# WeiZhang1988/YDORBSLAM

Hardware: AMD Instinct MI355X
Metric: ORB extract+match Mkeypoints/sec (higher is better)
Workload: dtype u8

## Files before the change

### ydorbslam_amd/csrc/match_kernels.hip.h

```cpp
#pragma once
#include <hip/hip_runtime.h>
#include <stdint.h>

#include <type_traits>

#include "grid_build.hip.h"

#pragma clang fp contract(off)

namespace ydorb {

constexpr int kHistLen = 30, kThHigh = 100, kThLow = 50;

template <class T> using gptr = __attribute__((address_space(1))) T*;
template <class T> __device__ __forceinline__ gptr<T> G(T* p) { return (gptr<T>)p; }

struct QueryDev {
  float u, v, r;
  int minLevel, maxLevel;
  float ur, rs, angle;
  int level, flags;
};

__global__ __launch_bounds__(256) void k_grid_build(const FrameDev* __restrict__ frames, int cap) {
  __shared__ int hist[kGridCells];
  __shared__ int wsum[4];
  extern __shared__ int16_t cellOf[];
  const FrameDev F = frames[blockIdx.x];
  grid_build<true>(F, cap, hist, wsum, cellOf);
}

__device__ __forceinline__ int hamming256(const uint8_t* a, const uint8_t* b) {
  const uint4 a0 = *reinterpret_cast<const uint4*>(a), a1 = *reinterpret_cast<const uint4*>(a + 16);
  const uint4 b0 = *reinterpret_cast<const uint4*>(b), b1 = *reinterpret_cast<const uint4*>(b + 16);
  return __popc(a0.x ^ b0.x) + __popc(a0.y ^ b0.y) + __popc(a0.z ^ b0.z) + __popc(a0.w ^ b0.w) + __popc(a1.x ^ b1.x) +
         __popc(a1.y ^ b1.y) + __popc(a1.z ^ b1.z) + __popc(a1.w ^ b1.w);
}

struct CallDev {
  int frame;
  const KeyPointDev* tkps;
  const float* qAngle;
  const QueryDev* queries;
  const uint8_t* qdesc;
  const int* nqPtr;
  int nq;
  int2* qInfo;
  uint8_t* taken;
  int* assigned;
  int* matchQ;
  int* count;
  int mode;
  float ratio;
  int orbDist, checkOri;
  float invSigma2[8];
  const KeyPointDev* qkps;
  uint2* qPre;
  int takenClear;
};
__device__ __forceinline__ int call_nq(const CallDev& C) { return C.nqPtr ? *C.nqPtr : C.nq; }

__device__ __forceinline__ unsigned wave_min_u32(unsigned v) {
#define YD_DPP_MIN(ctrl, rmask) v = min(v, (unsigned)__builtin_amdgcn_update_dpp((int)v, (int)v, ctrl, rmask, 0xF, false))
  YD_DPP_MIN(0xB1, 0xF);
  YD_DPP_MIN(0x4E, 0xF);
  YD_DPP_MIN(0x141, 0xF);
  YD_DPP_MIN(0x140, 0xF);
  YD_DPP_MIN(0x142, 0xA);
  YD_DPP_MIN(0x143, 0xC);
#undef YD_DPP_MIN
  return (unsigned)__builtin_amdgcn_readlane((int)v, 63);
}

constexpr int kSlot = 64;
#ifndef GATHER_QPW
#define GATHER_QPW 1
#endif
constexpr int kGatherQpw = GATHER_QPW;
__global__ __launch_bounds__(256) void k_gather_projection(const CallDev* __restrict__ calls, const FrameDev* __restrict__ frames,
                                                           int maxQ, uint32_t* __restrict__ pool, unsigned* __restrict__ poolHeads,
                                                           unsigned poolPerCall, int* __restrict__ status) {
  __shared__ int pref[4][64];
  __shared__ int sStart[4][64];
  const int lane = threadIdx.x & 63, wv = threadIdx.x >> 6;
  const int q0 = (blockIdx.x * 4 + wv) * kGatherQpw;
  const CallDev C = calls[blockIdx.y];
  const int nqAll = min(maxQ, call_nq(C));
  if (q0 >= nqAll) return;
  const FrameDev F = frames[C.frame];
  QueryDev Qs[kGatherQpw];
#pragma unroll
  for (int i = 0; i < kGatherQpw; i++) Qs[i] = C.queries[min(q0 + i, nqAll - 1)];
  struct Window { bool ok; int nx, start, cnt; };
  auto window = [&](const QueryDev& Q) -> Window {
    Window W{false, 0, 0, 0};
    if (!(Q.flags & 1)) return W;
    const int minCellX = max(0, (int)floorf(__fmul_rn(__fsub_rn(__fsub_rn(Q.u, F.minX), Q.r), F.gridWInv)));
    const int maxCellX = min(kGridCols - 1, (int)ceilf(__fmul_rn(__fadd_rn(__fsub_rn(Q.u, F.minX), Q.r), F.gridWInv)));
    const int minCellY = max(0, (int)floorf(__fmul_rn(__fsub_rn(__fsub_rn(Q.v, F.minY), Q.r), F.gridHInv)));
    const int maxCellY = min(kGridRows - 1, (int)ceilf(__fmul_rn(__fadd_rn(__fsub_rn(Q.v, F.minY), Q.r), F.gridHInv)));
    if (!(minCellX < kGridCols && maxCellX >= 0 && minCellY < kGridRows && maxCellY >= 0 && minCellX <= maxCellX && minCellY <= maxCellY)) return W;
    W.ok = true;
    W.nx = maxCellX - minCellX + 1;
    if (lane < W.nx) {
      const int c0 = (minCellX + lane) * kGridRows;
      W.start = F.cellStart[c0 + minCellY];
      W.cnt = F.cellStart[c0 + maxCellY + 1] - W.start;
    }
    return W;
  };
  Window Wn = window(Qs[0]);
#pragma unroll
  for (int qi = 0; qi < kGatherQpw; qi++) {
  const int q = q0 + qi;
  if (q >= nqAll) break;
  const QueryDev Q = Qs[qi];
  const Window Wc = Wn;
  if (qi + 1 < kGatherQpw && q + 1 < nqAll) Wn = window(Qs[qi + 1]);
  int2 info = make_int2(0, 0);
  if (Wc.ok) {
    {
      const int nx = Wc.nx;
      const int start = Wc.start, cnt = Wc.cnt;
      int incl = cnt;
#pragma unroll
      for (int d = 1; d < 64; d <<= 1) { const int y = __shfl_up(incl, d, 64); if (lane >= d) incl += y; }
      const int total = __shfl(incl, 63, 64);
      if (total > 0) {
        pref[wv][lane] = incl;
        sStart[wv][lane] = start;
        __builtin_amdgcn_wave_barrier();
        auto staticTest = [&](int t, int& pos, int& idx) -> bool {
          int lo = 0, hi = nx - 1;
          while (lo < hi) { const int mid = (lo + hi) >> 1; if (pref[wv][mid] > t) hi = mid; else lo = mid + 1; }
          pos = sStart[wv][lo] + (t - (lo ? pref[wv][lo - 1] : 0));
          const float4 kp = F.sortedKp[pos];
          const int octave = __float_as_int(kp.z);
          idx = __float_as_int(kp.w);
          bool pass = true;
          if (Q.minLevel > 0 || Q.maxLevel >= 0)
            if (octave < Q.minLevel || (Q.maxLevel >= 0 && octave < Q.maxLevel)) pass = false;
          if (!(fabsf(__fsub_rn(kp.x, Q.u)) > Q.r && fabsf(__fsub_rn(kp.y, Q.v)) < Q.r)) pass = false;
          if (pass && C.mode == 6) {
            const float rx = F.rightX ? F.rightX[idx] : -1.0f;
            const double ax = (double)__fsub_rn(kp.x, Q.u), ay = (double)__fsub_rn(kp.y, Q.v), ar = (double)__fsub_rn(rx, Q.ur);
            const float monoErr = (float)(ax * ax + ay * ay);
            const float stereoErr = (float)((double)monoErr + ar * ar);
            const bool lv = octave >= Q.level - 1 && octave <= Q.level;
            const float is2 = calls[blockIdx.y].invSigma2[octave & 7];
            pass = lv && ((rx >= 0 && (double)__fmul_rn(stereoErr, is2) <= 7.81) || (rx < 0 && (double)__fmul_rn(monoErr, is2) <= 5.99));
          } else if (pass && C.mode == 7) {
            pass = octave >= Q.level - 1 && octave <= Q.level;
          } else if (pass && C.mode != 2 && F.rightX) {
            const float rx = F.rightX[idx];
            if (!(rx <= 0 || fabsf(__fsub_rn(Q.ur, rx)) <= Q.rs)) pass = false;
          }
          return pass;
        };
        int need = total;
        if (total > kSlot) {
          need = 0;
          for (int t0 = 0; t0 < total; t0 += 64) {
            const int t = t0 + lane;
            int pos, idx;
            const bool pass = t < total && staticTest(t, pos, idx);
            need += __popcll(__ballot(pass));
          }
        }
        unsigned base;
        bool ok = true;
        if (need <= kSlot) {
          base = blockIdx.y * poolPerCall + (unsigned)q * kSlot;
        } else {
          unsigned off = 0;
          if (lane == 0) off = atomicAdd(poolHeads + blockIdx.y, (unsigned)need);
          off = __shfl(off, 0, 64);
          const unsigned ovfBase = (unsigned)maxQ * kSlot;
          ok = ovfBase + off + (unsigned)need <= poolPerCall;
          base = blockIdx.y * poolPerCall + ovfBase + off;
          if (!ok && lane == 0) atomicMax(status, 1);
        }
        if (ok && need > 0) {
          int written = 0;
          unsigned k1 = 0xFFFFFFFFu, k2 = 0xFFFFFFFFu, r1 = 0, r2 = 0;
          const bool pre = C.qPre != nullptr, readTaken = pre && C.taken && !C.takenClear;
          const uint4* qd = reinterpret_cast<const uint4*>(C.qdesc + (size_t)q * 32);
          const uint4 qa = qd[0], qb = qd[1];
          for (int t0 = 0; t0 < total; t0 += 64) {
            const int t = t0 + lane;
            int pos = 0, idx = 0, dist = 0;
            const bool pass = t < total && staticTest(t, pos, idx);
            if (pass) {
              const uint4* td = reinterpret_cast<const uint4*>(F.sortedDesc + (size_t)pos * 32);
              const uint4 ta = td[0], tb = td[1];
              dist = __popc(qa.x ^ ta.x) + __popc(qa.y ^ ta.y) + __popc(qa.z ^ ta.z) + __popc(qa.w ^ ta.w) + __popc(qb.x ^ tb.x) +
                     __popc(qb.y ^ tb.y) + __popc(qb.z ^ tb.z) + __popc(qb.w ^ tb.w);
            }
            const unsigned long long m = __ballot(pass);
            if (pass) {
              const int wpos = written + __popcll(m & ((1ull << lane) - 1ull));
              const uint32_t rec = ((uint32_t)dist << 16) | (uint32_t)idx;
              pool[base + wpos] = rec;
              if (pre && !(readTaken && C.taken[idx])) {
                const unsigned key = ((unsigned)dist << 23) | (unsigned)wpos;
                if (key < k1) { k2 = k1; r2 = r1; k1 = key; r1 = rec; } else if (key < k2) { k2 = key; r2 = rec; }
              }
            }
            written += __popcll(m);
          }
          if (pre) {
            const unsigned b1 = wave_min_u32(k1);
            const bool own = k1 == b1 && b1 != 0xFFFFFFFFu;
            const unsigned long long o1 = __ballot(own);
            const unsigned br = o1 ? (unsigned)__builtin_amdgcn_readlane((int)r1, (int)__builtin_ctzll(o1)) : 0xFFFFFFFFu;
            if (own) { k1 = k2; r1 = r2; }
            const unsigned b2 = wave_min_u32(k1);
            const unsigned long long o2 = __ballot(k1 == b2 && b2 != 0xFFFFFFFFu);
            const unsigned sr = o2 ? (unsigned)__builtin_amdgcn_readlane((int)r1, (int)__builtin_ctzll(o2)) : 0xFFFFFFFFu;
            if (lane == 0) C.qPre[q] = make_uint2(o1 ? br : 0xFFFFFFFFu, sr);
          }
          info = make_int2((int)base, written);
        }
      }
    }
  }
  if (lane == 0) C.qInfo[q] = info;
  __builtin_amdgcn_wave_barrier();
  }
}

struct BowCallDev {
  const uint8_t* descA; const uint8_t* descB;
  const int* qFeat; const int2* qRange; const int* featB; const uint8_t* validB;
  int nq;
  int2* qInfo;
  int tri;
  const KeyPointDev* kpsA; const KeyPointDev* kpsB;
  const uint8_t* goodA; const uint8_t* goodB;
  float F[9], ex, ey, sfB[8], sf2B[8];
};
__device__ __forceinline__ bool tri_pair_ok(const BowCallDev& B, const KeyPointDev& k1, bool good1, const KeyPointDev& k2, bool good2) {
  if (!(good1 || good2)) {
    const float dx = __fsub_rn(B.ex, k2.x), dy = __fsub_rn(B.ey, k2.y);
    const double far = (double)dx * (double)dx + (double)dy * (double)dy;
    if (!(far >= (double)__fmul_rn(100.0f, B.sfB[k2.octave]))) return false;
  }
  const float la = __fadd_rn(__fadd_rn(__fmul_rn(B.F[0], k1.x), __fmul_rn(B.F[3], k1.y)), B.F[6]);
  const float lb = __fadd_rn(__fadd_rn(__fmul_rn(B.F[1], k1.x), __fmul_rn(B.F[4], k1.y)), B.F[7]);
  const float lc = __fadd_rn(__fadd_rn(__fmul_rn(B.F[2], k1.x), __fmul_rn(B.F[5], k1.y)), B.F[8]);
  const float den = __fadd_rn(__fmul_rn(la, la), __fmul_rn(lb, lb));
  if (!(den > 0.0f)) return false;
  const float num = __fadd_rn(__fadd_rn(__fmul_rn(la, k2.x), __fmul_rn(lb, k2.y)), lc);
  return (double)__fdiv_rn(__fmul_rn(num, num), __fmul_rn(den, den)) < 3.841 * (double)B.sf2B[k2.octave];
}
__global__ __launch_bounds__(256) void k_gather_bow(BowCallDev B, uint32_t* __restrict__ pool, unsigned* __restrict__ poolHead,
                                                    unsigned poolCap, int* __restrict__ status) {
  const int lane = threadIdx.x & 63, wv = threadIdx.x >> 6;
  const int q = blockIdx.x * 4 + wv;
  if (q >= B.nq) return;
  const int2 rg = B.qRange[q];
  const int total = rg.y - rg.x;
  int2 info = make_int2(0, 0);
  if (total > 0) {
    unsigned base = 0;
    if (lane == 0) base = atomicAdd(poolHead, (unsigned)total);
    base = __shfl(base, 0, 64);
    if (base + (unsigned)total > poolCap) {
      if (lane == 0) atomicMax(status, 1);
    } else {
      const uint8_t* qd = B.descA + (size_t)B.qFeat[q] * 32;
      int written = 0;
      for (int t0 = 0; t0 < total; t0 += 64) {
        const int t = t0 + lane;
        bool pass = false;
        int idx = 0, dist = 0;
        if (t < total) {
          idx = B.featB[rg.x + t];
          pass = !B.validB || B.validB[idx];
          if (pass) dist = hamming256(qd, B.descB + (size_t)idx * 32);
          if (pass && B.tri) {
            const int i1 = B.qFeat[q];
            pass = dist <= kThLow && tri_pair_ok(B, B.kpsA[i1], B.goodA[i1] != 0, B.kpsB[idx], B.goodB[idx] != 0);
          }
        }
        const unsigned long long m = __ballot(pass);
        if (pass) pool[base + written + __popcll(m & ((1ull << lane) - 1ull))] = ((uint32_t)dist << 16) | (uint32_t)idx;
        written += __popcll(m);
      }
      info = make_int2((int)base, written);
    }
  }
  if (lane == 0) B.qInfo[q] = info;
}


__global__ __launch_bounds__(256) void k_distinctive(const uint8_t* __restrict__ desc, const int* __restrict__ offsets, int nPoints,
                                                     int* __restrict__ best) {
  const int p = blockIdx.x * 4 + (threadIdx.x >> 6), lane = threadIdx.x & 63;
  if (p >= nPoints) return;
  const int o0 = __builtin_amdgcn_readfirstlane(offsets[p]), m = __builtin_amdgcn_readfirstlane(offsets[p + 1]) - o0;
  if (m <= 0) { if (lane == 0) best[p] = -1; return; }
  const uint8_t* D = desc + (size_t)o0 * 32;
  const int kth = (int)(0.5 * m);
  unsigned win = 0xFFFFFFFFu;
  for (int i0 = 0; i0 < m; i0 += 64) {
    const int i = i0 + lane;
    if (i < m) {
      const uint4 a0 = *reinterpret_cast<const uint4*>(D + (size_t)i * 32), a1 = *reinterpret_cast<const uint4*>(D + (size_t)i * 32 + 16);
      int lo = 0, hi = 256;
      while (lo < hi) {
// ... 403 lines not shown
```

### ydorbslam_amd/csrc/orb_matcher.hip

```cpp
#include <hip/hip_runtime.h>

#include <algorithm>
#include <cstdlib>
#include <cmath>
#include <cstring>
#include <vector>

#include "../../include/ydorb/c_api.h"
#include "frustum_kernels.hip.h"
#include "host_buffers.h"
#include "match_kernels.hip.h"
#include "stereo_kernels.hip.h"
#include "ydorb_host.h"

using namespace ydorb;

namespace {

int launchGridBuild(int nFrames, int cap, hipStream_t s, const FrameDev* frames) {
  const size_t dyn = sizeof(int16_t) * (size_t)std::max(cap, 0);
  if (dyn > 48 * 1024)
    HIPCHK(hipFuncSetAttribute(reinterpret_cast<const void*>(k_grid_build), hipFuncAttributeMaxDynamicSharedMemorySize, (int)dyn));
  hipLaunchKernelGGL(k_grid_build, dim3(nFrames), dim3(256), dyn, s, frames, cap);
  HIPCHK(hipGetLastError());
// ... 35 lines not shown
struct ProjPtrs {
  int* status; FrameDev* frame; CallDev* call;
  KeyPointDev* kps; uint8_t* desc; float* rightX; int *cellStart, *cellIdx; float4* sortedKp; uint8_t* sortedDesc;
  QueryDev* queries; uint8_t *qdesc, *taken; int *assigned, *matchQ; int2* qInfo; uint2* qPre;
  uint8_t *table, *track;
};
size_t layProjection(size_t n, bool stereo, size_t nq, size_t tableBytes, size_t trackBytes, void* base, ProjPtrs& p) {
  Carve a(base);
  a.take(p.status, 16); a.take(p.frame, 1); a.take(p.call, 1);
  a.take(p.kps, n); a.take(p.desc, 32 * n); a.take(p.rightX, stereo ? n : 0); a.take(p.cellStart, kGridCells + 1); a.take(p.cellIdx, n);
  a.take(p.sortedKp, n); a.take(p.sortedDesc, 32 * n);
  a.take(p.queries, nq); a.take(p.qdesc, 32 * nq); a.take(p.taken, n + kTakenPad); a.take(p.assigned, n); a.take(p.matchQ, nq); a.take(p.qInfo, nq);
  a.take(p.qPre, nq); a.take(p.table, tableBytes); a.take(p.track, trackBytes);
  return a.L.bytes;
}

struct BowPtrs {
  int* status; CallDev* call;
  uint8_t *descA, *descB, *valid, *goodA, *goodB; KeyPointDev *kpsA, *kpsB; int *feat, *qFeat, *assigned, *matchQ; int2 *qRange, *qInfo; float* qAngle;
};
size_t layBow(size_t nA, size_t nB, size_t nFeatB, size_t nq, bool tri, void* base, BowPtrs& p) {
  Carve a(base);
  a.take(p.status, 16); a.take(p.call, 1);
  a.take(p.descA, 32 * nA); a.take(p.descB, 32 * nB); a.take(p.kpsB, nB); a.take(p.feat, nFeatB); a.take(p.valid, nB);
  a.take(p.qFeat, nq); a.take(p.qRange, nq); a.take(p.qAngle, nq); a.take(p.qInfo, nq); a.take(p.matchQ, nq); a.take(p.assigned, std::max(nq, nB));
  a.take(p.kpsA, tri ? nA : 0); a.take(p.goodA, tri ? nA : 0); a.take(p.goodB, tri ? nB : 0);
  return a.L.bytes;
}

struct RowsPtrs { uint8_t *a, *b; int *offsets, *idx, *out; TopkOut* top; };
size_t layRows(size_t nA, size_t nB, size_t nOffsets, size_t nIdx, size_t nOut, size_t nTop, void* base, RowsPtrs& r) {
  Carve a(base);
  a.take(r.a, 32 * nA); a.take(r.b, 32 * nB); a.take(r.offsets, nOffsets); a.take(r.idx, nIdx); a.take(r.out, nOut); a.take(r.top, nTop);
  return a.L.bytes;
}

struct StereoPtrs { int *counters, *kept, *status, *nL, *nR; KeyPointDev *kpsL, *kpsR; uint8_t *descL, *descR; float *rightX, *depth; };
size_t layStereo(size_t nPairs, size_t nl, size_t nr, void* base, StereoPtrs& p) {
  Carve a(base);
  a.take(p.counters, 4 * nPairs); a.take(p.kept, nPairs); a.take(p.status, nPairs);
  a.take(p.kpsL, nl); a.take(p.descL, 32 * nl); a.take(p.kpsR, nr); a.take(p.descR, 32 * nr); a.take(p.nL, nl ? nPairs : 0); a.take(p.nR, nl ? nPairs : 0);
  a.take(p.rightX, nl); a.take(p.depth, nl);
  return a.L.bytes;
}

}

struct ydorb_matcher {
  int device = 0;
  hipStream_t stream = nullptr;
  Mem call;
  Mem pool;
  size_t poolRecords = 1u << 20;
  Mem stereo;
  PinnedMem hUp, hDown;
  struct Batch {
    Mem arena;
    Mem status;
    std::vector<FrameDev> hFrames;
    std::vector<CallDev> hCalls;
    float hSf[8] = {0};
    bool hIdentAffine = false;
    BatchPtrs at{};
    int ovfPerKeypoint = 16;
  } batch;
  bool profiling = false;
  hipEvent_t ev[MS_COUNT + 1]{};
  double stageMs[MS_COUNT]{};
  int stageCalls = 0;
  bool evPending = false;
  std::vector<Mem*> buffers() { return {&call, &pool, &stereo, &hUp, &hDown, &batch.arena, &batch.status}; }
  ydorb_matcher() { for (Mem* b : buffers()) b->slackDiv = 2; }
};

static void collect(ydorb_matcher* m) {
  if (!m->profiling || !m->evPending) return;
  m->evPending = false;
  if (hipEventQuery(m->ev[MS_COUNT]) != hipSuccess) return;
  for (int i = 0; i < MS_COUNT; i++) {
    float ms = 0;
    if (hipEventElapsedTime(&ms, m->ev[i], m->ev[i + 1]) == hipSuccess) m->stageMs[i] += ms;
  }
  m->stageCalls++;
}

static bool validFrameView(const YdFrameView* fv) {
  return fv && fv->n >= 0 && (fv->n == 0 || (fv->kps && fv->desc)) && fv->max_x > fv->min_x && fv->max_y > fv->min_y;
}

extern "C" {

void ydorb_matcher_destroy(ydorb_matcher_t* m) {
  if (!m) return;
  (void)hipSetDevice(m->device);
  (void)hipStreamSynchronize(m->stream);
  for (Mem* b : m->buffers()) b->release();
  for (auto& e : m->ev) if (e) (void)hipEventDestroy(e);
  (void)hipStreamDestroy(m->stream);
  delete m;
}

int ydorb_matcher_create(int32_t device, ydorb_matcher_t** out) {
  if (!out) { set_error("null argument"); return YDORB_ERR_INVALID_ARG; }
  *out = nullptr;
  int rc = require_device(device);
  if (rc) return rc;
  ydorb_matcher* m = new ydorb_matcher();
  m->device = device;
  if (hipStreamCreateWithFlags(&m->stream, hipStreamNonBlocking) != hipSuccess) {
    set_error("hipStreamCreate failed");
    delete m;
    return YDORB_ERR_HIP;
  }
  for (auto& e : m->ev) (void)hipEventCreate(&e);
  if (m->batch.status.ensure(64) != YDORB_OK || hipMemset(m->batch.status.p, 0, 64) != hipSuccess) {
    set_error("matcher scratch allocation failed");
    ydorb_matcher_destroy(m);
    return YDORB_ERR_HIP;
  }
  *out = m;
  return YDORB_OK;
}

int ydorb_descriptor_distance(const uint8_t* a, const uint8_t* b) {
  int d = 0;
  for (int i = 0; i < 32; i += 8) {
    uint64_t x, y;
    memcpy(&x, a + i, 8);
    memcpy(&y, b + i, 8);
    d += __builtin_popcountll(x ^ y);
  }
  return d;
}

int ydorb_descriptor_distance_rows(ydorb_matcher_t* m, const uint8_t* a, const uint8_t* b, int32_t n, int32_t* out) {
  if (!m || !a || !b || !out || n < 0) { set_error("invalid argument"); return YDORB_ERR_INVALID_ARG; }
  if (n == 0) return YDORB_OK;
  HIPCHK(hipSetDevice(m->device));
  RowsPtrs r;
  if (const int rc = layOut(m->call, [&](void* base) { return layRows(n, n, 0, 0, n, 0, base, r); })) return rc;
  HIPCHK(hipMemcpyAsync(r.a, a, (size_t)32 * n, hipMemcpyHostToDevice, m->stream));
  HIPCHK(hipMemcpyAsync(r.b, b, (size_t)32 * n, hipMemcpyHostToDevice, m->stream));
  hipLaunchKernelGGL(k_hamming_rows, dim3((n + 255) / 256), dim3(256), 0, m->stream, r.a, r.b, n, r.out);
  HIPCHK(hipMemcpyAsync(out, r.out, sizeof(int) * n, hipMemcpyDeviceToHost, m->stream));
  HIPCHK(hipStreamSynchronize(m->stream));
  return YDORB_OK;
}

int ydorb_distinctive_descriptors(ydorb_matcher_t* m, const uint8_t* desc, const int32_t* offsets, int32_t nPoints, int32_t* best) {
  if (!m || !offsets || !best || nPoints < 0) { set_error("invalid argument"); return YDORB_ERR_INVALID_ARG; }
  if (nPoints == 0) return YDORB_OK;
  const int total = offsets[nPoints];
  if (offsets[0] != 0 || total < 0 || (total > 0 && !desc)) { set_error("invalid offsets"); return YDORB_ERR_INVALID_ARG; }
  for (int p = 0; p < nPoints; p++) {
    const int cnt = offsets[p + 1] - offsets[p];
    if (cnt < 0 || cnt > 65535) { set_error("map point %d holds %d descriptors (0..65535 supported)", p, cnt); return YDORB_ERR_INVALID_ARG; }
  }
  HIPCHK(hipSetDevice(m->device));
  RowsPtrs r;
  if (const int rc = layOut(m->call, [&](void* base) { return layRows(std::max(total, 1), 0, nPoints + 1, 0, nPoints, 0, base, r); })) return rc;
  if (total) HIPCHK(hipMemcpyAsync(r.a, desc, (size_t)32 * total, hipMemcpyHostToDevice, m->stream));
  HIPCHK(hipMemcpyAsync(r.offsets, offsets, sizeof(int) * (nPoints + 1), hipMemcpyHostToDevice, m->stream));
  hipLaunchKernelGGL(k_distinctive, dim3((nPoints + 3) / 4), dim3(256), 0, m->stream, r.a, r.offsets, nPoints, r.out);
  HIPCHK(hipGetLastError());
  HIPCHK(hipMemcpyAsync(best, r.out, sizeof(int) * nPoints, hipMemcpyDeviceToHost, m->stream));
  HIPCHK(hipStreamSynchronize(m->stream));
  return YDORB_OK;
}

static int searchProjectionImpl(ydorb_matcher_t* m, int32_t mode, const YdFrameView* fv, const YdQuery* queries, const uint8_t* qdesc,
                                int32_t nq, float ratio, int32_t orbDist, int32_t checkOri, uint8_t* taken, int32_t* assigned,
                                int32_t* nMatches, std::vector<uint32_t>* recordsOut, const float* invSigma2 = nullptr, int nLevels = 0,
                                int32_t* bestOut = nullptr, const ProjPtrs* laid = nullptr) {
  HIPCHK(hipSetDevice(m->device));
  const int n = fv->n;
  if (n > 65535) { set_error("frames with more than 65535 keypoints are not supported"); return YDORB_ERR_UNSUPPORTED; }
  if (nq == 0 || n == 0) { *nMatches = 0; return YDORB_OK; }
  int rc;
  ProjPtrs p;
  if (laid) p = *laid;
  else if ((rc = layOut(m->call, [&](void* base) { return layProjection(n, fv->right_x, nq, 0, 0, base, p); }))) return rc;
  for (int attempt = 0; attempt < 6; attempt++) {
    const size_t poolCap = (size_t)nq * kSlot + m->poolRecords;
    if ((rc = m->pool.ensure(sizeof(uint32_t) * poolCap))) return rc;
    HIPCHK(hipMemcpyAsync(p.kps, fv->kps, sizeof(YdKeyPoint) * n, hipMemcpyHostToDevice, m->stream));
    HIPCHK(hipMemcpyAsync(p.desc, fv->desc, (size_t)32 * n, hipMemcpyHostToDevice, m->stream));
    if (fv->right_x) HIPCHK(hipMemcpyAsync(p.rightX, fv->right_x, sizeof(float) * n, hipMemcpyHostToDevice, m->stream));
    FrameDev F{};
    F.kps = p.kps; F.desc = p.desc; F.rightX = fv->right_x ? p.rightX : nullptr; F.nPtr = nullptr; F.n = n;
    F.minX = fv->min_x; F.minY = fv->min_y;
    F.gridWInv = static_cast<float>(kGridCols) / (fv->max_x - fv->min_x);
    F.gridHInv = static_cast<float>(kGridRows) / (fv->max_y - fv->min_y);
    F.cellStart = p.cellStart; F.cellIdx = p.cellIdx; F.sortedKp = p.sortedKp; F.sortedDesc = p.sortedDesc;
    HIPCHK(hipMemcpyAsync(p.frame, &F, sizeof(FrameDev), hipMemcpyHostToDevice, m->stream));
    if ((rc = launchGridBuild(1, n, m->stream, p.frame))) return rc;
    HIPCHK(hipMemsetAsync(p.status, 0, 64, m->stream));
    if (queries) HIPCHK(hipMemcpyAsync(p.queries, queries, sizeof(YdQuery) * nq, hipMemcpyHostToDevice, m->stream));
    HIPCHK(hipMemcpyAsync(p.qdesc, qdesc, (size_t)32 * nq, hipMemcpyHostToDevice, m->stream));
    if (taken) HIPCHK(hipMemcpyAsync(p.taken, taken, n, hipMemcpyHostToDevice, m->stream));
    else HIPCHK(hipMemsetAsync(p.taken, 0, n, m->stream));
    if (assigned) HIPCHK(hipMemcpyAsync(p.assigned, assigned, sizeof(int) * n, hipMemcpyHostToDevice, m->stream));
    CallDev C{};
    C.tkps = p.kps; C.queries = p.queries; C.qdesc = p.qdesc; C.nq = nq; C.qInfo = p.qInfo; C.qPre = p.qPre;
    C.taken = p.taken; C.takenClear = taken ? 0 : 1; C.assigned = p.assigned; C.matchQ = p.matchQ;
    C.count = p.status + 2; C.mode = mode; C.ratio = ratio; C.orbDist = orbDist; C.checkOri = checkOri;
    for (int i = 0; i < 8; i++) C.invSigma2[i] = (invSigma2 && i < nLevels) ? invSigma2[i] : 0.f;
    HIPCHK(hipMemcpyAsync(p.call, &C, sizeof(CallDev), hipMemcpyHostToDevice, m->stream));
    hipLaunchKernelGGL(k_gather_projection, dim3((nq + 4 * kGatherQpw - 1) / (4 * kGatherQpw), 1), dim3(256), 0, m->stream, p.call, p.frame, nq,
                       m->pool.as<uint32_t>(), reinterpret_cast<unsigned*>(p.status), (unsigned)poolCap, p.status + 1);
    int hmisc[3];
    if (!recordsOut) {
      const int takenWords = (n + 31) / 32;
      hipLaunchKernelGGL(k_resolve, dim3(1), dim3(64), 2 * sizeof(unsigned) * takenWords, m->stream, p.call, p.frame, m->pool.as<uint32_t>(), takenWords);
    }
    HIPCHK(hipGetLastError());
    HIPCHK(hipMemcpyAsync(hmisc, p.status, sizeof(hmisc), hipMemcpyDeviceToHost, m->stream));
    HIPCHK(hipStreamSynchronize(m->stream));
    if (hmisc[1] != 0) {
      m->poolRecords = std::max<size_t>(m->poolRecords * 4, (size_t)(unsigned)hmisc[0] + 1024);
      continue;
    }
    if (recordsOut) {
      std::vector<int2> info(nq);
      HIPCHK(hipMemcpy(info.data(), p.qInfo, sizeof(int2) * nq, hipMemcpyDeviceToHost));
      recordsOut->resize(info[0].y);
      if (info[0].y) HIPCHK(hipMemcpy(recordsOut->data(), m->pool.as<uint32_t>() + info[0].x, sizeof(uint32_t) * info[0].y, hipMemcpyDeviceToHost));
      return YDORB_OK;
    }
    if (taken) HIPCHK(hipMemcpy(taken, p.taken, n, hipMemcpyDeviceToHost));
    if (assigned) HIPCHK(hipMemcpy(assigned, p.assigned, sizeof(int) * n, hipMemcpyDeviceToHost));
    if (bestOut) HIPCHK(hipMemcpy(bestOut, p.matchQ, sizeof(int) * nq, hipMemcpyDeviceToHost));
    *nMatches = hmisc[2];
    return YDORB_OK;
  }
  set_error("candidate record pool kept overflowing");
  return YDORB_ERR_CAPACITY;
}

struct BowJob {
  struct Side {
    const YdKeyPoint* kps; const uint8_t* desc; int n; const YdFeatureVector* fv;
    const uint8_t* ok;
    const uint8_t* good;
  } A, B;
  int mode;
  float ratio;
  int checkOri;
  BowCallDev geom;
};

static int bowSearch(ydorb_matcher_t* m, const BowJob& J, std::vector<int>& qFeat, std::vector<int>& res, int32_t* nMatches) {
  std::vector<int2> qRange;
  std::vector<float> qAngle;
  size_t records = 0;
  const YdFeatureVector &fa = *J.A.fv, &fb = *J.B.fv;
  for (int a = 0, b = 0; a < fa.n_nodes && b < fb.n_nodes;) {
    if (fa.node_ids[a] == fb.node_ids[b]) {
      for (int ia = fa.node_start[a]; ia < fa.node_start[a + 1]; ia++) {
        const int idxA = fa.feat[ia];
        if (!J.A.ok[idxA]) continue;
        qFeat.push_back(idxA);
        qRange.push_back(make_int2(fb.node_start[b], fb.node_start[b + 1]));
        qAngle.push_back(J.A.kps[idxA].angle);
        records += (size_t)(fb.node_start[b + 1] - fb.node_start[b]);
      }
      a++; b++;
    } else if (fa.node_ids[a] < fb.node_ids[b]) {
      a = (int)(std::lower_bound(fa.node_ids, fa.node_ids + fa.n_nodes, fb.node_ids[b]) - fa.node_ids);
    } else {
      b = (int)(std::lower_bound(fb.node_ids, fb.node_ids + fb.n_nodes, fa.node_ids[a]) - fb.node_ids);
    }
  }
  const int nq = (int)qFeat.size();
  if (nq == 0) return YDORB_OK;
  const int nFeatB = fb.node_start[fb.n_nodes], nA = J.A.n, nB = J.B.n;
  m->poolRecords = std::max<size_t>(m->poolRecords, records + 1024);
  int rc;
  BowPtrs p;
  if ((rc = layOut(m->call, [&](void* base) { return layBow(nA, nB, std::max(nFeatB, 1), nq, J.geom.tri, base, p); })) ||
      (rc = m->pool.ensure(sizeof(uint32_t) * m->poolRecords)))
    return rc;
  hipStream_t s = m->stream;
  HIPCHK(hipMemsetAsync(p.status, 0, 64, s));
  HIPCHK(hipMemcpyAsync(p.descA, J.A.desc, (size_t)32 * nA, hipMemcpyHostToDevice, s));
  HIPCHK(hipMemcpyAsync(p.descB, J.B.desc, (size_t)32 * nB, hipMemcpyHostToDevice, s));
  HIPCHK(hipMemcpyAsync(p.kpsB, J.B.kps, sizeof(YdKeyPoint) * nB, hipMemcpyHostToDevice, s));
  if (nFeatB) HIPCHK(hipMemcpyAsync(p.feat, fb.feat, sizeof(int) * nFeatB, hipMemcpyHostToDevice, s));
  if (J.B.ok) HIPCHK(hipMemcpyAsync(p.valid, J.B.ok, nB, hipMemcpyHostToDevice, s));
  HIPCHK(hipMemcpyAsync(p.qFeat, qFeat.data(), sizeof(int) * nq, hipMemcpyHostToDevice, s));
  HIPCHK(hipMemcpyAsync(p.qRange, qRange.data(), sizeof(int2) * nq, hipMemcpyHostToDevice, s));
  HIPCHK(hipMemcpyAsync(p.qAngle, qAngle.data(), sizeof(float) * nq, hipMemcpyHostToDevice, s));
// ... 275 lines not shown
int ydorb_match_pairs_device(ydorb_matcher_t* m, const YdFrameSetDev* Q, const YdFrameSetDev* T, const int32_t* pairs, int32_t nCalls,
                             int32_t width, int32_t height, float th, const float* scaleFactors, int32_t nLevels, const float* d_affine,
                             int32_t checkOri, int32_t* d_assigned, int32_t* d_counts, void* stream) {
  if (!m || !Q || !T || !pairs || !Q->d_kps || !Q->d_desc || !Q->d_n || !T->d_kps || !T->d_desc || !T->d_n || !d_assigned || !d_counts || !scaleFactors ||
      Q->cap < 1 || Q->cap > 65535 || T->cap != Q->cap || Q->n_frames < 1 || T->n_frames < 1 || nCalls < 1 || nLevels < 1 || nLevels > 8 || width < 1 ||
      height < 1) {
    set_error("invalid argument");
    return YDORB_ERR_INVALID_ARG;
  }
  for (int c = 0; c < nCalls; c++)
    if (pairs[2 * c] < 0 || pairs[2 * c] >= Q->n_frames || pairs[2 * c + 1] < 0 || pairs[2 * c + 1] >= T->n_frames) {
      set_error("pair %d references a frame out of range", c);
      return YDORB_ERR_INVALID_ARG;
    }
  HIPCHK(hipSetDevice(m->device));
  hipStream_t s = stream ? (hipStream_t)stream : m->stream;
  std::vector<int> tmap(T->n_frames, -1);
  std::vector<int> tused;
  for (int c = 0; c < nCalls; c++) {
    const int tf = pairs[2 * c + 1];
    if (tmap[tf] < 0) { tmap[tf] = (int)tused.size(); tused.push_back(tf); }
  }
  auto& B = m->batch;
  const int cap = Q->cap, nFrames = (int)tused.size();
  const size_t poolPerCall = (size_t)cap * kSlot + (size_t)cap * B.ovfPerKeypoint;
  BatchPtrs p;
  const size_t had = B.arena.cap;
  const int rc = layOut(B.arena, [&](void* base) { return layBatch(cap, nCalls, nFrames, poolPerCall, base, p); });
  if (B.arena.cap != had) B.hFrames.clear();
  if (rc) return rc;
  std::vector<FrameDev> hf(nFrames);
  std::vector<CallDev> hc(nCalls);
  const float minX = 0.f, minY = 0.f, maxX = (float)width, maxY = (float)height;
  for (int f = 0; f < nFrames; f++) {
    const int tf = tused[f];
    FrameDev& F = hf[f];
    F.kps = reinterpret_cast<const KeyPointDev*>(T->d_kps) + (size_t)tf * cap; F.desc = T->d_desc + (size_t)tf * cap * 32; F.rightX = nullptr;
    F.nPtr = T->d_n + tf; F.n = 0; F.minX = minX; F.minY = minY;
    F.gridWInv = static_cast<float>(kGridCols) / (maxX - minX); F.gridHInv = static_cast<float>(kGridRows) / (maxY - minY);
    F.cellStart = p.cellStart + (size_t)f * (kGridCells + 1); F.cellIdx = p.cellIdx + (size_t)f * cap;
    F.sortedKp = p.sortedKp + (size_t)f * cap; F.sortedDesc = p.sortedDesc + (size_t)f * cap * 32;
  }
  for (int c = 0; c < nCalls; c++) {
    const int qf = pairs[2 * c], tf = tmap[pairs[2 * c + 1]];
    CallDev& C = hc[c];
    C.frame = tf; C.tkps = hf[tf].kps; C.qAngle = nullptr; C.queries = p.queries + (size_t)c * cap;
    C.qkps = reinterpret_cast<const KeyPointDev*>(Q->d_kps) + (size_t)qf * cap;
    C.qdesc = Q->d_desc + (size_t)qf * cap * 32; C.nqPtr = Q->d_n + qf; C.nq = 0; C.qInfo = p.qInfo + (size_t)c * cap;
    C.qPre = p.qPre + (size_t)c * cap; C.takenClear = 1;
    C.taken = p.taken + (size_t)c * cap; C.assigned = d_assigned + (size_t)c * cap; C.matchQ = p.matchQ + (size_t)c * cap;
    C.count = d_counts + c; C.mode = 1; C.ratio = 0.9f; C.orbDist = 0; C.checkOri = checkOri;
  }
  float hsf[8] = {0};
  for (int l = 0; l < nLevels; l++) hsf[l] = scaleFactors[l];
  const bool same = p.frames == B.at.frames && p.calls == B.at.calls && p.sf == B.at.sf && p.ident == B.at.ident &&
                    B.hFrames.size() == hf.size() && B.hCalls.size() == hc.size() && !memcmp(B.hFrames.data(), hf.data(), sizeof(FrameDev) * hf.size()) &&
                    !memcmp(B.hCalls.data(), hc.data(), sizeof(CallDev) * hc.size()) && !memcmp(B.hSf, hsf, sizeof(hsf)) && B.hIdentAffine == !d_affine;
  if (!same) {
    HIPCHK(hipStreamSynchronize(s));
    B.hFrames.clear();
    HIPCHK(hipMemcpy(p.frames, hf.data(), sizeof(FrameDev) * nFrames, hipMemcpyHostToDevice));
    HIPCHK(hipMemcpy(p.calls, hc.data(), sizeof(CallDev) * nCalls, hipMemcpyHostToDevice));
    HIPCHK(hipMemcpy(p.sf, hsf, sizeof(hsf), hipMemcpyHostToDevice));
    if (!d_affine) {
      std::vector<float> ident((size_t)6 * nCalls, 0.f);
      for (int c = 0; c < nCalls; c++) { ident[6 * c] = 1.f; ident[6 * c + 4] = 1.f; }
      HIPCHK(hipMemcpy(p.ident, ident.data(), sizeof(float) * ident.size(), hipMemcpyHostToDevice));
    }
    B.hFrames.swap(hf);
    B.hCalls.swap(hc);
    memcpy(B.hSf, hsf, sizeof(hsf));
    B.hIdentAffine = !d_affine;
    B.at = p;
  }
  const float* aff = d_affine ? d_affine : p.ident;
  const bool prof = m->profiling;
  collect(m);
  int* const ovf = B.status.as<int>() + 1;
  if (prof) HIPCHK(hipEventRecord(m->ev[0], s));
  hipLaunchKernelGGL(k_queries_from_keypoints, dim3((cap + 255) / 256, nCalls), dim3(256), 0, s, p.calls, cap, aff, th, p.sf, nLevels, minX, maxX, minY, maxY,
                     p.heads);
  { const int rcg = launchGridBuild(nFrames, cap, s, p.frames); if (rcg) return rcg; }
  if (prof) HIPCHK(hipEventRecord(m->ev[1], s));
  hipLaunchKernelGGL(k_gather_projection, dim3((cap + 4 * kGatherQpw - 1) / (4 * kGatherQpw), nCalls), dim3(256), 0, s, p.calls, p.frames, cap, p.pool, p.heads,
                     (unsigned)poolPerCall, ovf);
  if (prof) HIPCHK(hipEventRecord(m->ev[2], s));
  const int takenWords = (cap + 31) / 32;
  hipLaunchKernelGGL(k_resolve, dim3(nCalls), dim3(64), 2 * sizeof(unsigned) * takenWords, s, p.calls, p.frames, p.pool, takenWords);
  if (prof) { HIPCHK(hipEventRecord(m->ev[3], s)); m->evPending = true; }
  HIPCHK(hipGetLastError());
  return YDORB_OK;
}

int ydorb_match_consecutive_device(ydorb_matcher_t* m, const YdKeyPoint* d_kps, const uint8_t* d_desc, const int32_t* d_n, int32_t cap,
                                   int32_t nFrames, int32_t width, int32_t height, float th, const float* scaleFactors, int32_t nLevels,
                                   const float* d_affine, int32_t checkOri, int32_t* d_assigned, int32_t* d_counts, void* stream) {
  if (!m || nFrames < 2) { set_error("invalid argument"); return YDORB_ERR_INVALID_ARG; }
  const YdFrameSetDev S{d_kps, d_desc, d_n, nFrames, cap};
  std::vector<int32_t> pairs((size_t)2 * (nFrames - 1));
  for (int c = 0; c < nFrames - 1; c++) { pairs[2 * c] = c; pairs[2 * c + 1] = c + 1; }
  return ydorb_match_pairs_device(m, &S, &S, pairs.data(), nFrames - 1, width, height, th, scaleFactors, nLevels, d_affine, checkOri, d_assigned,
                                  d_counts, stream);
}

int ydorb_hamming_topk(ydorb_matcher_t* m, const uint8_t* q, int32_t nq, const uint8_t* t, int32_t nt, const int32_t* candOffsets,
                       const int32_t* candIdx, YdMatch2* out) {
  static_assert(sizeof(YdMatch2) == sizeof(TopkOut), "YdMatch2 layout");
  if (!m || nq < 0 || nt < 0 || nt > 65535 || (nq && (!q || !out)) || (nt && !t) || ((candOffsets == nullptr) != (candIdx == nullptr))) {
    set_error("invalid argument");
    return YDORB_ERR_INVALID_ARG;
  }
  if (nq == 0) return YDORB_OK;
  int rc = require_device(m->device);
  if (rc) return rc;
  HIPCHK(hipSetDevice(m->device));
  size_t nCand = 0;
  if (candOffsets) {
    if (candOffsets[0] != 0) { set_error("cand_offsets[0] must be 0"); return YDORB_ERR_INVALID_ARG; }
    for (int i = 0; i < nq; i++) {
      const int n = candOffsets[i + 1] - candOffsets[i];
      if (n < 0 || n > 65535) { set_error("candidate list %d has %d entries (0..65535 supported)", i, n); return YDORB_ERR_INVALID_ARG; }
    }
    nCand = (size_t)candOffsets[nq];
  }
  hipStream_t s = m->stream;
  RowsPtrs r;
  if ((rc = layOut(m->call, [&](void* base) { return layRows(nq, std::max(nt, 1), (size_t)nq + 1, std::max<size_t>(nCand, 1), 0, nq, base, r); }))) return rc;
  HIPCHK(hipMemcpyAsync(r.a, q, (size_t)32 * nq, hipMemcpyHostToDevice, s));
  if (nt) HIPCHK(hipMemcpyAsync(r.b, t, (size_t)32 * nt, hipMemcpyHostToDevice, s));
  if (candOffsets) {
    HIPCHK(hipMemcpyAsync(r.offsets, candOffsets, sizeof(int) * ((size_t)nq + 1), hipMemcpyHostToDevice, s));
    if (nCand) HIPCHK(hipMemcpyAsync(r.idx, candIdx, sizeof(int) * nCand, hipMemcpyHostToDevice, s));
  }
  hipLaunchKernelGGL(k_topk_csr, dim3((nq + 3) / 4), dim3(256), 0, s, r.a, nq, r.b, nt, candOffsets ? r.offsets : nullptr, candOffsets ? r.idx : nullptr, r.top);
  HIPCHK(hipGetLastError());
  HIPCHK(hipMemcpyAsync(out, r.top, sizeof(TopkOut) * (size_t)nq, hipMemcpyDeviceToHost, s));
  HIPCHK(hipStreamSynchronize(s));
  return YDORB_OK;
}

int ydorb_hamming_topk_device(ydorb_matcher_t* m, const uint8_t* d_qdesc, const int32_t* d_nq, const uint8_t* d_tdesc, const int32_t* d_nt, int32_t cap,
                              int32_t nPairs, YdMatch2* d_out, void* stream) {
  if (!m || !d_qdesc || !d_nq || !d_tdesc || !d_nt || !d_out || cap < 1 || cap > 65535 || nPairs < 1) { set_error("invalid argument"); return YDORB_ERR_INVALID_ARG; }
  int rc = require_device(m->device);
  if (rc) return rc;
  HIPCHK(hipSetDevice(m->device));
  hipStream_t s = stream ? (hipStream_t)stream : m->stream;
  hipLaunchKernelGGL(k_topk_allpairs, dim3((cap + 255) / 256, nPairs), dim3(256), 0, s, d_qdesc, d_nq, (size_t)cap * 32, d_tdesc, d_nt, (size_t)cap * 32, cap,
                     reinterpret_cast<TopkOut*>(d_out));
  HIPCHK(hipGetLastError());
  return YDORB_OK;
}

int ydorb_matcher_synchronize(ydorb_matcher_t* m) {
  if (!m) { set_error("null handle"); return YDORB_ERR_INVALID_ARG; }
  HIPCHK(hipSetDevice(m->device));
  HIPCHK(hipDeviceSynchronize());
  collect(m);
  if (Mem& st = m->batch.status; st.p) {
    int hmisc[2];
    HIPCHK(hipMemcpy(hmisc, st.p, sizeof(hmisc), hipMemcpyDeviceToHost));
    if (hmisc[1] != 0) {
      (void)hipMemset(st.p, 0, 8);
      m->batch.ovfPerKeypoint *= 4;
      set_error("candidate record pool overflow in the batched search: results of that call are incomplete; the overflow region is now %d records per keypoint, call again",
                m->batch.ovfPerKeypoint);
      return YDORB_ERR_CAPACITY;
    }
// ... 26 lines not shown
```

Baseline: 182.7.

## Stage grid cell offsets in LDS and prefetch queries in gather kernel

Refactors the projection-gather body into a templated per-query routine. It adds a staged kernel in which each block copies the whole cellStart table into shared memory and processes 64 queries per block, prefetching the next query and its descriptor one iteration ahead. It also replaces the shuffle-based prefix scan with a DPP-based scan, reads queries through scalar constant-address loads, and tags global pointers with an explicit address space. The staged path is chosen by default when there are multiple calls. The cost is a larger LDS footprint and fewer blocks in flight per call.

```diff
diff --git a/ydorbslam_amd/csrc/match_kernels.hip.h b/ydorbslam_amd/csrc/match_kernels.hip.h
--- a/ydorbslam_amd/csrc/match_kernels.hip.h
+++ b/ydorbslam_amd/csrc/match_kernels.hip.h
@@ -14,6 +14,8 @@
 
 template <class T> using gptr = __attribute__((address_space(1))) T*;
 template <class T> __device__ __forceinline__ gptr<T> G(T* p) { return (gptr<T>)p; }
+template <class T> using kptr = __attribute__((address_space(4))) T*;
+template <class T> __device__ __forceinline__ kptr<T> K(T* p) { return (kptr<T>)p; }
 
 struct QueryDev {
   float u, v, r;
@@ -72,69 +74,85 @@
   return (unsigned)__builtin_amdgcn_readlane((int)v, 63);
 }
 
+__device__ __forceinline__ int wave_incl_scan_i32(int v) {
+#define YD_DPP_ADD(ctrl, rmask) v += __builtin_amdgcn_update_dpp(0, v, ctrl, rmask, 0xF, false)
+  YD_DPP_ADD(0x111, 0xF);
+  YD_DPP_ADD(0x112, 0xF);
+  YD_DPP_ADD(0x114, 0xF);
+  YD_DPP_ADD(0x118, 0xF);
+  YD_DPP_ADD(0x142, 0xA);
+  YD_DPP_ADD(0x143, 0xC);
+#undef YD_DPP_ADD
+  return v;
+}
+
+__device__ __forceinline__ QueryDev load_query_uniform(const QueryDev* qp) {
+  static_assert(sizeof(QueryDev) == 40, "QueryDev is read as 10 dwords");
+  const auto w = K(reinterpret_cast<const unsigned*>(qp));
+  QueryDev Q;
+  Q.u = __uint_as_float(w[0]); Q.v = __uint_as_float(w[1]); Q.r = __uint_as_float(w[2]);
+  Q.minLevel = (int)w[3]; Q.maxLevel = (int)w[4];
+  Q.ur = __uint_as_float(w[5]); Q.rs = __uint_as_float(w[6]); Q.angle = __uint_as_float(w[7]);
+  Q.level = (int)w[8]; Q.flags = (int)w[9];
+  return Q;
+}
+
 constexpr int kSlot = 64;
-#ifndef GATHER_QPW
-#define GATHER_QPW 1
-#endif
-constexpr int kGatherQpw = GATHER_QPW;
-__global__ __launch_bounds__(256) void k_gather_projection(const CallDev* __restrict__ calls, const FrameDev* __restrict__ frames,
-                                                           int maxQ, uint32_t* __restrict__ pool, unsigned* __restrict__ poolHeads,
-                                                           unsigned poolPerCall, int* __restrict__ status) {
-  __shared__ int pref[4][64];
-  __shared__ int sStart[4][64];
-  const int lane = threadIdx.x & 63, wv = threadIdx.x >> 6;
-  const int q0 = (blockIdx.x * 4 + wv) * kGatherQpw;
-  const CallDev C = calls[blockIdx.y];
-  const int nqAll = min(maxQ, call_nq(C));
-  if (q0 >= nqAll) return;
-  const FrameDev F = frames[C.frame];
-  QueryDev Qs[kGatherQpw];
-#pragma unroll
-  for (int i = 0; i < kGatherQpw; i++) Qs[i] = C.queries[min(q0 + i, nqAll - 1)];
-  struct Window { bool ok; int nx, start, cnt; };
-  auto window = [&](const QueryDev& Q) -> Window {
-    Window W{false, 0, 0, 0};
-    if (!(Q.flags & 1)) return W;
+
+typedef float v4f __attribute__((ext_vector_type(4)));
+typedef unsigned v4u __attribute__((ext_vector_type(4)));
+typedef unsigned v2u __attribute__((ext_vector_type(2)));
+typedef int v2i __attribute__((ext_vector_type(2)));
+
+struct GatherFromHbm {
+  gptr<const int> cells; gptr<const v4f> kps; kptr<const v4u> qd;
+  __device__ __forceinline__ int cell(int i) const { return cells[i]; }
+  __device__ __forceinline__ v4f kp(int pos) const { return kps[pos]; }
+  __device__ __forceinline__ void qdesc(int q, v4u& a, v4u& b) const { a = qd[2 * (size_t)q]; b = qd[2 * (size_t)q + 1]; }
+};
+struct GatherStaged {
+  const int* cells; gptr<const v4f> kps; v4u qa, qb;
+  __device__ __forceinline__ int cell(int i) const { return cells[i]; }
+  __device__ __forceinline__ v4f kp(int pos) const { return kps[pos]; }
+  __device__ __forceinline__ void qdesc(int, v4u& a, v4u& b) const { a = qa; b = qb; }
+};
+
+template <class Src>
+__device__ __forceinline__ void gather_one_query(const Src& S, const CallDev* __restrict__ calls, int call, const CallDev& C, const FrameDev& F,
+                                                 int q, const QueryDev& Q, int lane, int* pref, int* sStart, int maxQ,
+                                                 uint32_t* __restrict__ pool, unsigned* __restrict__ poolHeads, unsigned poolPerCall,
+                                                 int* __restrict__ status) {
+  bool inGrid = false;
+  int nx = 0, start = 0, cnt = 0;
+  if (Q.flags & 1) {
     const int minCellX = max(0, (int)floorf(__fmul_rn(__fsub_rn(__fsub_rn(Q.u, F.minX), Q.r), F.gridWInv)));
     const int maxCellX = min(kGridCols - 1, (int)ceilf(__fmul_rn(__fadd_rn(__fsub_rn(Q.u, F.minX), Q.r), F.gridWInv)));
     const int minCellY = max(0, (int)floorf(__fmul_rn(__fsub_rn(__fsub_rn(Q.v, F.minY), Q.r), F.gridHInv)));
     const int maxCellY = min(kGridRows - 1, (int)ceilf(__fmul_rn(__fadd_rn(__fsub_rn(Q.v, F.minY), Q.r), F.gridHInv)));
-    if (!(minCellX < kGridCols && maxCellX >= 0 && minCellY < kGridRows && maxCellY >= 0 && minCellX <= maxCellX && minCellY <= maxCellY)) return W;
-    W.ok = true;
-    W.nx = maxCellX - minCellX + 1;
-    if (lane < W.nx) {
-      const int c0 = (minCellX + lane) * kGridRows;
-      W.start = F.cellStart[c0 + minCellY];
-      W.cnt = F.cellStart[c0 + maxCellY + 1] - W.start;
-    }
-    return W;
-  };
-  Window Wn = window(Qs[0]);
-#pragma unroll
-  for (int qi = 0; qi < kGatherQpw; qi++) {
-  const int q = q0 + qi;
-  if (q >= nqAll) break;
-  const QueryDev Q = Qs[qi];
-  const Window Wc = Wn;
-  if (qi + 1 < kGatherQpw && q + 1 < nqAll) Wn = window(Qs[qi + 1]);
+    if (minCellX < kGridCols && maxCellX >= 0 && minCellY < kGridRows && maxCellY >= 0 && minCellX <= maxCellX && minCellY <= maxCellY) {
+      inGrid = true;
+      nx = maxCellX - minCellX + 1;
+      if (lane < nx) {
+        const int c0 = (minCellX + lane) * kGridRows;
+        start = S.cell(c0 + minCellY);
+        cnt = S.cell(c0 + maxCellY + 1) - start;
+      }
+    }
+  }
   int2 info = make_int2(0, 0);
-  if (Wc.ok) {
+  if (inGrid) {
     {
-      const int nx = Wc.nx;
-      const int start = Wc.start, cnt = Wc.cnt;
-      int incl = cnt;
-#pragma unroll
-      for (int d = 1; d < 64; d <<= 1) { const int y = __shfl_up(incl, d, 64); if (lane >= d) incl += y; }
-      const int total = __shfl(incl, 63, 64);
+      const int incl = wave_incl_scan_i32(cnt);
+      const int total = __builtin_amdgcn_readlane(incl, 63);
       if (total > 0) {
-        pref[wv][lane] = incl;
-        sStart[wv][lane] = start;
+        pref[lane] = incl;
+        sStart[lane] = start;
         __builtin_amdgcn_wave_barrier();
         auto staticTest = [&](int t, int& pos, int& idx) -> bool {
           int lo = 0, hi = nx - 1;
-          while (lo < hi) { const int mid = (lo + hi) >> 1; if (pref[wv][mid] > t) hi = mid; else lo = mid + 1; }
-          pos = sStart[wv][lo] + (t - (lo ? pref[wv][lo - 1] : 0));
-          const float4 kp = F.sortedKp[pos];
+          while (lo < hi) { const int mid = (lo + hi) >> 1; if (pref[mid] > t) hi = mid; else lo = mid + 1; }
+          pos = sStart[lo] + (t - (lo ? pref[lo - 1] : 0));
+          const v4f kp = S.kp(pos);
           const int octave = __float_as_int(kp.z);
           idx = __float_as_int(kp.w);
           bool pass = true;
@@ -142,17 +160,17 @@
             if (octave < Q.minLevel || (Q.maxLevel >= 0 && octave < Q.maxLevel)) pass = false;
           if (!(fabsf(__fsub_rn(kp.x, Q.u)) > Q.r && fabsf(__fsub_rn(kp.y, Q.v)) < Q.r)) pass = false;
           if (pass && C.mode == 6) {
-            const float rx = F.rightX ? F.rightX[idx] : -1.0f;
+            const float rx = F.rightX ? G(F.rightX)[idx] : -1.0f;
             const double ax = (double)__fsub_rn(kp.x, Q.u), ay = (double)__fsub_rn(kp.y, Q.v), ar = (double)__fsub_rn(rx, Q.ur);
             const float monoErr = (float)(ax * ax + ay * ay);
             const float stereoErr = (float)((double)monoErr + ar * ar);
             const bool lv = octave >= Q.level - 1 && octave <= Q.level;
-            const float is2 = calls[blockIdx.y].invSigma2[octave & 7];
+            const float is2 = calls[call].invSigma2[octave & 7];
             pass = lv && ((rx >= 0 && (double)__fmul_rn(stereoErr, is2) <= 7.81) || (rx < 0 && (double)__fmul_rn(monoErr, is2) <= 5.99));
           } else if (pass && C.mode == 7) {
             pass = octave >= Q.level - 1 && octave <= Q.level;
           } else if (pass && C.mode != 2 && F.rightX) {
-            const float rx = F.rightX[idx];
+            const float rx = G(F.rightX)[idx];
             if (!(rx <= 0 || fabsf(__fsub_rn(Q.ur, rx)) <= Q.rs)) pass = false;
           }
           return pass;
@@ -170,29 +188,29 @@
         unsigned base;
         bool ok = true;
         if (need <= kSlot) {
-          base = blockIdx.y * poolPerCall + (unsigned)q * kSlot;
+          base = call * poolPerCall + (unsigned)q * kSlot;
         } else {
           unsigned off = 0;
-          if (lane == 0) off = atomicAdd(poolHeads + blockIdx.y, (unsigned)need);
+          if (lane == 0) off = atomicAdd(poolHeads + call, (unsigned)need);
           off = __shfl(off, 0, 64);
           const unsigned ovfBase = (unsigned)maxQ * kSlot;
           ok = ovfBase + off + (unsigned)need <= poolPerCall;
-          base = blockIdx.y * poolPerCall + ovfBase + off;
+          base = call * poolPerCall + ovfBase + off;
           if (!ok && lane == 0) atomicMax(status, 1);
         }
         if (ok && need > 0) {
           int written = 0;
           unsigned k1 = 0xFFFFFFFFu, k2 = 0xFFFFFFFFu, r1 = 0, r2 = 0;
           const bool pre = C.qPre != nullptr, readTaken = pre && C.taken && !C.takenClear;
-          const uint4* qd = reinterpret_cast<const uint4*>(C.qdesc + (size_t)q * 32);
-          const uint4 qa = qd[0], qb = qd[1];
+          v4u qa, qb;
+          S.qdesc(q, qa, qb);
           for (int t0 = 0; t0 < total; t0 += 64) {
             const int t = t0 + lane;
             int pos = 0, idx = 0, dist = 0;
             const bool pass = t < total && staticTest(t, pos, idx);
             if (pass) {
-              const uint4* td = reinterpret_cast<const uint4*>(F.sortedDesc + (size_t)pos * 32);
-              const uint4 ta = td[0], tb = td[1];
+              const auto td = G(reinterpret_cast<const v4u*>(F.sortedDesc + (size_t)pos * 32));
+              const v4u ta = td[0], tb = td[1];
               dist = __popc(qa.x ^ ta.x) + __popc(qa.y ^ ta.y) + __popc(qa.z ^ ta.z) + __popc(qa.w ^ ta.w) + __popc(qb.x ^ tb.x) +
                      __popc(qb.y ^ tb.y) + __popc(qb.z ^ tb.z) + __popc(qb.w ^ tb.w);
             }
@@ -201,7 +219,7 @@
               const int wpos = written + __popcll(m & ((1ull << lane) - 1ull));
               const uint32_t rec = ((uint32_t)dist << 16) | (uint32_t)idx;
               pool[base + wpos] = rec;
-              if (pre && !(readTaken && C.taken[idx])) {
+              if (pre && !(readTaken && G(C.taken)[idx])) {
                 const unsigned key = ((unsigned)dist << 23) | (unsigned)wpos;
                 if (key < k1) { k2 = k1; r2 = r1; k1 = key; r1 = rec; } else if (key < k2) { k2 = key; r2 = rec; }
               }
@@ -217,15 +235,62 @@
             const unsigned b2 = wave_min_u32(k1);
             const unsigned long long o2 = __ballot(k1 == b2 && b2 != 0xFFFFFFFFu);
             const unsigned sr = o2 ? (unsigned)__builtin_amdgcn_readlane((int)r1, (int)__builtin_ctzll(o2)) : 0xFFFFFFFFu;
-            if (lane == 0) C.qPre[q] = make_uint2(o1 ? br : 0xFFFFFFFFu, sr);
+            if (lane == 0) G(reinterpret_cast<v2u*>(C.qPre))[q] = v2u{o1 ? br : 0xFFFFFFFFu, sr};
           }
           info = make_int2((int)base, written);
         }
       }
     }
   }
-  if (lane == 0) C.qInfo[q] = info;
+  if (lane == 0) G(reinterpret_cast<v2i*>(C.qInfo))[q] = v2i{info.x, info.y};
   __builtin_amdgcn_wave_barrier();
+}
+
+__global__ __launch_bounds__(256) void k_gather_projection(const CallDev* __restrict__ calls, const FrameDev* __restrict__ frames,
+                                                           int maxQ, uint32_t* __restrict__ pool, unsigned* __restrict__ poolHeads,
+                                                           unsigned poolPerCall, int* __restrict__ status) {
+  __shared__ int pref[4][64];
+  __shared__ int sStart[4][64];
+  const int lane = threadIdx.x & 63, wv = __builtin_amdgcn_readfirstlane(threadIdx.x >> 6);
+  const int q = blockIdx.x * 4 + wv;
+  const CallDev C = calls[blockIdx.y];
+  const int nqAll = min(maxQ, call_nq(C));
+  if (q >= nqAll) return;
+  const FrameDev F = frames[C.frame];
+  const QueryDev Q = load_query_uniform(C.queries + q);
+  const GatherFromHbm S{G(const_cast<const int*>(F.cellStart)), G(reinterpret_cast<const v4f*>(F.sortedKp)), K(reinterpret_cast<const v4u*>(C.qdesc))};
+  gather_one_query(S, calls, (int)blockIdx.y, C, F, q, Q, lane, pref[wv], sStart[wv], maxQ, pool, poolHeads, poolPerCall, status);
+}
+
+constexpr int kGatherChunk = 64;
+__global__ __launch_bounds__(256) void k_gather_projection_staged(const CallDev* __restrict__ calls, const FrameDev* __restrict__ frames,
+                                                                  int maxQ, uint32_t* __restrict__ pool, unsigned* __restrict__ poolHeads,
+                                                                  unsigned poolPerCall, int* __restrict__ status) {
+  __shared__ int pref[4][64];
+  __shared__ int sStart[4][64];
+  __shared__ int sCell[kGridCells + 1];
+  const int lane = threadIdx.x & 63, wv = __builtin_amdgcn_readfirstlane(threadIdx.x >> 6);
+  const int call = blockIdx.y, q0 = blockIdx.x * kGatherChunk;
+  const CallDev C = calls[call];
+  const int nqAll = min(maxQ, call_nq(C));
+  if (q0 >= nqAll) return;
+  const int qEnd = min(nqAll, q0 + kGatherChunk);
+  const FrameDev F = frames[C.frame];
+  struct Ahead { QueryDev Q; v4u a, b; };
+  auto request = [&](int q) -> Ahead {
+    const auto d = K(reinterpret_cast<const v4u*>(C.qdesc + (size_t)q * 32));
+    return Ahead{load_query_uniform(C.queries + q), d[0], d[1]};
+  };
+  Ahead next{};
+  if (q0 + wv < qEnd) next = request(q0 + wv);
+  const auto cs = G(const_cast<const int*>(F.cellStart));
+  for (int i = threadIdx.x; i <= kGridCells; i += 256) sCell[i] = cs[i];
+  __syncthreads();
+  for (int q = q0 + wv; q < qEnd; q += 4) {
+    const Ahead cur = next;
+    if (q + 4 < qEnd) next = request(q + 4);
+    const GatherStaged S{sCell, G(reinterpret_cast<const v4f*>(F.sortedKp)), cur.a, cur.b};
+    gather_one_query(S, calls, call, C, F, q, cur.Q, lane, pref[wv], sStart[wv], maxQ, pool, poolHeads, poolPerCall, status);
   }
 }
 
diff --git a/ydorbslam_amd/csrc/orb_matcher.hip b/ydorbslam_amd/csrc/orb_matcher.hip
--- a/ydorbslam_amd/csrc/orb_matcher.hip
+++ b/ydorbslam_amd/csrc/orb_matcher.hip
@@ -141,6 +141,16 @@
     if (hipEventElapsedTime(&ms, m->ev[i], m->ev[i + 1]) == hipSuccess) m->stageMs[i] += ms;
   }
   m->stageCalls++;
+}
+
+static void launchBatchGather(int nCalls, int cap, hipStream_t s, const BatchPtrs& p, unsigned poolPerCall, int* ovf) {
+  const char* sel = getenv("YDORB_GATHER_STAGED");
+  const bool staged = sel ? atoi(sel) != 0 : nCalls > 1;
+  if (staged)
+    hipLaunchKernelGGL(k_gather_projection_staged, dim3((cap + kGatherChunk - 1) / kGatherChunk, nCalls), dim3(256), 0, s, p.calls, p.frames, cap, p.pool,
+                       p.heads, poolPerCall, ovf);
+  else
+    hipLaunchKernelGGL(k_gather_projection, dim3((cap + 3) / 4, nCalls), dim3(256), 0, s, p.calls, p.frames, cap, p.pool, p.heads, poolPerCall, ovf);
 }
 
 static bool validFrameView(const YdFrameView* fv) {
@@ -265,7 +275,7 @@
     C.count = p.status + 2; C.mode = mode; C.ratio = ratio; C.orbDist = orbDist; C.checkOri = checkOri;
     for (int i = 0; i < 8; i++) C.invSigma2[i] = (invSigma2 && i < nLevels) ? invSigma2[i] : 0.f;
     HIPCHK(hipMemcpyAsync(p.call, &C, sizeof(CallDev), hipMemcpyHostToDevice, m->stream));
-    hipLaunchKernelGGL(k_gather_projection, dim3((nq + 4 * kGatherQpw - 1) / (4 * kGatherQpw), 1), dim3(256), 0, m->stream, p.call, p.frame, nq,
+    hipLaunchKernelGGL(k_gather_projection, dim3((nq + 3) / 4, 1), dim3(256), 0, m->stream, p.call, p.frame, nq,
                        m->pool.as<uint32_t>(), reinterpret_cast<unsigned*>(p.status), (unsigned)poolCap, p.status + 1);
     int hmisc[3];
     if (!recordsOut) {
@@ -707,8 +717,7 @@
                      p.heads);
   { const int rcg = launchGridBuild(nFrames, cap, s, p.frames); if (rcg) return rcg; }
   if (prof) HIPCHK(hipEventRecord(m->ev[1], s));
-  hipLaunchKernelGGL(k_gather_projection, dim3((cap + 4 * kGatherQpw - 1) / (4 * kGatherQpw), nCalls), dim3(256), 0, s, p.calls, p.frames, cap, p.pool, p.heads,
-                     (unsigned)poolPerCall, ovf);
+  launchBatchGather(nCalls, cap, s, p, (unsigned)poolPerCall, ovf);
   if (prof) HIPCHK(hipEventRecord(m->ev[2], s));
   const int takenWords = (cap + 31) / 32;
   hipLaunchKernelGGL(k_resolve, dim3(nCalls), dim3(64), 2 * sizeof(unsigned) * takenWords, s, p.calls, p.frames, p.pool, takenWords);
```

After: 181.0. About the same (-1.0%).
